# shenwei356/wfa

Measured on AMD Instinct MI355X. Metric: aligned pairs/sec (and Gcells/s) on 1e6 synthetic 1 kbp pairs @5% error, higher is better.
Workload: dtype u32; 1 GPU; 1000000 x 1000 bp pairs/GPU @5% error, global gap-affine 4/6/2, wf-adaptive 10/50/1, seed 3; config=c3, pairs_per_gpu=1000000, length=1000, parallelism=pair-sharded x1, ranks_seen_by_collective=1, backend=none (1 GPU), collective_forced=False, status_ok=1000000, setup_steps=0, gather=none (1 GPU), gather_bytes_per_rank_step=0, packed_pairs=1000000, retried_pairs=831

## Files before the change

### wfa_amd/csrc/wfa_duo.hpp

```cpp
#pragma once
#include "wfa_blk.hpp"
#include "wfa_duo_cfg.hpp"
#include "wfa_pk16.hpp"

namespace wfa {

struct DuoRed {
#define WFA_DUO_3(opa, opb, opc)                                                                                    \
    unsigned long long sv;                                                                                          \
    asm volatile("s_nop 1\n\t" opa " %0, %0, %0 " WFA_DPP_CTL_XOR1 "\n\t" opb " %1, %1, %1 " WFA_DPP_CTL_XOR1 "\n\t" opc \
        " %2, %2, %2 " WFA_DPP_CTL_XOR1 "\n\t" opa " %0, %0, %0 " WFA_DPP_CTL_XOR2 "\n\t" opb " %1, %1, %1 "        \
        WFA_DPP_CTL_XOR2 "\n\t" opc " %2, %2, %2 " WFA_DPP_CTL_XOR2 "\n\t" opa " %0, %0, %0 " WFA_DPP_CTL_HMIR "\n\t" \
        opb " %1, %1, %1 " WFA_DPP_CTL_HMIR "\n\t" opc " %2, %2, %2 " WFA_DPP_CTL_HMIR "\n\t"                         \
        "s_and_saveexec_b64 %3, %4\n\t" opa " %0, %0, %0 " WFA_DPP_CTL_MIR "\n\t" opb " %1, %1, %1 " WFA_DPP_CTL_MIR    \
        "\n\t" opc " %2, %2, %2 " WFA_DPP_CTL_MIR "\n\ts_mov_b64 exec, %3"                                            \
        : "+v"(a), "+v"(b), "+v"(c), "=&s"(sv)                                                                      \
        : "s"(wm)                                                                                                   \
        : "scc");
#define WFA_DUO_2(opa, opb)                                                                                         \
    unsigned long long sv;                                                                                          \
    asm volatile("s_nop 1\n\t" opa " %0, %0, %0 " WFA_DPP_CTL_XOR1 "\n\t" opb " %1, %1, %1 " WFA_DPP_CTL_XOR1 "\n\ts_nop 0\n\t" \
        opa " %0, %0, %0 " WFA_DPP_CTL_XOR2 "\n\t" opb " %1, %1, %1 " WFA_DPP_CTL_XOR2 "\n\ts_nop 0\n\t" opa        \
        " %0, %0, %0 " WFA_DPP_CTL_HMIR "\n\t" opb " %1, %1, %1 " WFA_DPP_CTL_HMIR "\n\t"                            \
        "s_and_saveexec_b64 %2, %3\n\t" opa " %0, %0, %0 " WFA_DPP_CTL_MIR "\n\t" opb " %1, %1, %1 " WFA_DPP_CTL_MIR    \
// ... 29 lines not shown
__device__ __attribute__((always_inline)) inline void duo_run(const KParams &P) {
    constexpr int PP = 4;
    static_assert(DX >= 1 && DOE >= 1 && DX <= 4 && DOE <= 4, "ring depths of one to four score steps");
    constexpr int R  = DX > DOE ? DX : DOE;
    constexpr int RW = PK ? 2 : PP;
    extern __shared__ __attribute__((aligned(16))) uint32_t lds[];
    const int  lane = threadIdx.x, l7 = lane & 7, l15 = lane & 15;
    const bool hi_half = (lane & 8) != 0;

    const uint32_t  SW = P.lds_seq_words, PW = P.prepack_words;
    const uint32_t  FP = duo_fetch_pairs(PW), NBUF = duo_bufs(PW);
    uint32_t *const park0 = lds + NBUF * PW;
    const uint64_t  cap      = P.arena_words;
    const int       mdd      = (int)P.max_dist_diff;
    const int       minwf    = (int)P.min_wf_len;
    const bool      adaptive = P.adaptive != 0;
    const uint32_t  seed_si  = P.dx;
    uint32_t        pk_one   = 0x00010001u;
    if constexpr (PK) asm volatile("" : "+s"(pk_one));
    const int       rows_cap = (int)(cap / 32);

    int       st = 0;
    bool      wide = false;
    uint32_t  pidx = 0, si = 0, cells = 0, sbuf = 0;
    int       n = 0, m = 0, kb = 0;
    bool      slow = false, first_eq = false;
    int             j = l7, k0 = 0;
    uint32_t        mdn = 0u, mup = 0u;
    const uint32_t *lq = lds + 4, *lt = lds + 4;
    uint32_t       *rowp = nullptr;

    uint32_t M[R][RW], I[RW], D[RW];
    int      rlo[R], rhi[R];
    int      lim[PP], lmx[PP];
#pragma unroll
    for (int d = 0; d < R; d++) {
        rlo[d] = BK_BIG, rhi[d] = -BK_BIG;
#pragma unroll
        for (int p = 0; p < RW; p++) M[d][p] = 0u;
    }
#pragma unroll
    for (int p = 0; p < RW; p++) I[p] = D[p] = 0u;
#pragma unroll
    for (int p = 0; p < PP; p++) lim[p] = 0, lmx[p] = 0;

    uint32_t buf_free  = (1u << NBUF) - 1u;
    uint32_t park_used = 0u;
    constexpr uint32_t PF_TOK = 1u, PF_LD = 2u, PF_STAGED = 4u, PF_DRY = 8u;
    uint32_t pf = 0u;
    uint32_t pf_tok = 0u, pf_ld_idx = 0u, pf_idx = 0u, pf_buf = 0u;
    uint32_t st_mask = 0u;
    uint4    pf_w = make_uint4(0u, 0u, 0u, 0u);

#ifdef WFA_STAMPS
    unsigned long long stamp_acc[8] = {0, 0, 0, 0, 0, 0, 0, 0}, stamp_prev;
    unsigned long long evt[16] = {0, 0, 0, 0, 0, 0, 0, 0, 0, 0, 0, 0, 0, 0, 0, 0};
    asm volatile("s_memtime %0\n\ts_waitcnt lgkmcnt(0)" : "=s"(stamp_prev)::"memory");
#endif
    const auto pair_of = [&](uint32_t idx) { return P.work ? P.work[idx] : P.chunk_first + idx; };
    const auto dn1 = [&](uint32_t x) { return (uint32_t)__builtin_amdgcn_update_dpp(0, (int)x, 0x111, 0xf, 0xf, true) & mdn; };
    const auto up1 = [&](uint32_t x) { return (uint32_t)__builtin_amdgcn_update_dpp(0, (int)x, 0x101, 0xf, 0xf, true) & mup; };
    const auto other_half = [&](int x) { return __builtin_amdgcn_update_dpp(0, x, 0x128, 0xf, 0xf, true); };
    const auto set_derived = [&]() {
        j   = wide ? l15 : l7;
        mdn = j == 0 ? 0u : ~0u;
        mup = j == (wide ? 15 : 7) ? 0u : ~0u;
        k0  = kb + PP * j;
#pragma unroll
        for (int p = 0; p < PP; p++) lim[p] = imax2(1, imin2(n + k0 + p, m)), lmx[p] = imax2(n + k0 + p, m);
        lq   = lds + sbuf * PW + 4u;
        lt   = lq + SW;
        if constexpr (DUO_ARENA_FMT == 10u)
            rowp = P.arena + (uint64_t)pidx * cap + (((uint32_t)k0 & 56u) >> 3) * (uint32_t)(rows_cap * 4) + (((uint32_t)k0 >> 2) & 1u) * 16u;
        else if constexpr (DUO_ARENA_FMT == 9u)
            rowp = P.arena + (uint64_t)pidx * cap + (((uint32_t)k0 & 60u) >> 2) * (uint32_t)(rows_cap * 2) + si * 2u;
        else
            rowp = P.arena + (uint64_t)pidx * cap + (uint64_t)(si >> 3) * 256u + (si & 7u) * 2u;
    };
    const auto clear_rings = [&]() {
#pragma unroll
        for (int d = 0; d < R; d++) {
            rlo[d] = BK_BIG, rhi[d] = -BK_BIG;
#pragma unroll
            for (int p = 0; p < RW; p++) M[d][p] = 0u;
        }
#pragma unroll
        for (int p = 0; p < RW; p++) I[p] = D[p] = 0u;
    };
    const auto or_halves = [&](uint32_t v) {
        uint32_t r = 0u;
#pragma unroll
        for (int o = 0; o < 8; o++) r |= (uint32_t)__builtin_amdgcn_readlane((int)v, 8 * o);
        return r;
    };

    const auto refill = [&](auto ph_c) __attribute__((always_inline)) -> bool {
        constexpr int ph  = decltype(ph_c)::value;
        constexpr int NEW = (ph + R - 1) % R;
        pf        = (uint32_t)__builtin_amdgcn_readfirstlane((int)pf);
        park_used = (uint32_t)__builtin_amdgcn_readfirstlane((int)park_used);
        buf_free  = (uint32_t)__builtin_amdgcn_readfirstlane((int)buf_free);
        st_mask   = (uint32_t)__builtin_amdgcn_readfirstlane((int)st_mask);
        if ((pf & (PF_LD | PF_STAGED)) == PF_LD) {
            const uint32_t cnt = umin2(FP, P.chunk_n - pf_ld_idx);
            st_mask = 0u;
            {
                uint32_t f = buf_free;
                for (uint32_t c = 0; c < cnt; c++) st_mask |= f & (0u - f), f &= f - 1u;
            }
            buf_free &= ~st_mask;
            const uint32_t w0 = (uint32_t)lane * 4u, slot = w0 / PW;
            if (slot < cnt) {
                uint32_t f = st_mask;
                for (uint32_t c = 0; c < slot; c++) f &= f - 1u;
                const uint32_t b = (uint32_t)__builtin_ctz(f);
                *reinterpret_cast<uint4 *>(lds + b * PW + (w0 - slot * PW)) = pf_w;
            }
            pf_idx = pf_ld_idx, pf = (pf | PF_STAGED) & ~PF_LD;
        }
        if ((pf & (PF_TOK | PF_LD)) == PF_TOK) {
            pf_ld_idx = (uint32_t)__builtin_amdgcn_readfirstlane((int)pf_tok);
            const bool have = pf_ld_idx < P.chunk_n;
            if (have) {
                const uint32_t *const slot = P.prepack + (uint64_t)pf_ld_idx * PW;
                const uint32_t cnt = umin2(FP, P.chunk_n - pf_ld_idx);
                if ((uint32_t)lane * 4u < cnt * PW) pf_w = *reinterpret_cast<const uint4 *>(slot + lane * 4);
            }
            pf = (pf & ~PF_TOK) | (have ? PF_LD : PF_DRY);
        }
        if ((pf & (PF_TOK | PF_DRY)) == 0u) {
            if (lane == 0) pf_tok = atomicAdd(P.queue_head, FP);
            pf |= PF_TOK;
        }
        unsigned long long m_free;
        WFA_STAMP(0);
        for (;;) {
        const bool run   = st == 1;
        const int  Wc    = wide ? 64 : 32;
        const bool touch = run && rhi[NEW] >= rlo[NEW] && (rlo[NEW] <= kb || rhi[NEW] >= kb + Wc - 1);
        bool       narrowable = false;
        if constexpr (ph == 0) {
            int ulo = rlo[0], uhi = rhi[0];
#pragma unroll
            for (int d = 1; d < R; d++) ulo = imin2(ulo, rlo[d]), uhi = imax2(uhi, rhi[d]);
            narrowable    = run && wide && uhi - ulo + 1 <= DUO_NARROW_AT;
        }
        const unsigned long long m_ev = __ballot(touch || narrowable);
        m_free = __ballot(st == 0);
        if (__builtin_expect(!(m_ev != 0ull || (m_free != 0ull && (park_used != 0u || (pf & PF_STAGED) != 0u))), 1)) break;
        WFA_EVT(1, 1);
        {
            int ulo = rlo[0], uhi = rhi[0];
#pragma unroll
            for (int d = 1; d < R; d++) ulo = imin2(ulo, rlo[d]), uhi = imax2(uhi, rhi[d]);
            const int span = uhi - ulo + 1;
            int act = 0;
            if (touch) act = wide ? (span > DUO_WIDE_MAX ? 4 : 1) : (span > DUO_WIDEN_AT ? 2 : 1);
            else if (narrowable) act = 3;
            const int Wn  = act == 2 ? 64 : (act == 3 ? 32 : Wc);
            const int kbn = (((ulo + uhi + 1 - Wn) >> 1) + 2) & ~3;
            if (act != 0 && act != 4 && !(ulo - kbn >= 1 && uhi - kbn <= Wn - 2)) act = 4;
            const int  o_act = other_half(act), o_kb = other_half(kb), o_kbn = other_half(kbn);
            const bool o_wide = other_half(wide ? 1 : 0) != 0;
            bool widen  = act == 2 && !(hi_half && o_act == 2);
            bool taken  = !wide && !o_wide && o_act == 2 && !(!hi_half && act == 2);
            bool evict  = taken && st == 1;
            unsigned long long m_evict = __ballot(evict);
            bool               lost    = false;
            while (m_evict != 0ull) {
                const int      l0   = __builtin_ctzll(m_evict);
                const uint32_t oct  = (uint32_t)l0 >> 3;
                m_evict &= ~(0xFFull << (8 * oct));
                const bool mine = evict && ((uint32_t)lane >> 3) == oct;
                if (park_used == (1u << DUO_PARK) - 1u) {
                    if (((uint32_t)lane >> 3) == (oct ^ 1u)) lost = true;
                    if (mine) evict = false, taken = false;
                    continue;
                }
                const uint32_t rec = (uint32_t)__builtin_ctz(~park_used);
                park_used |= 1u << rec;
                WFA_EVT(3, 1);
                uint32_t *const pr = park0 + rec * DUO_PARK_WORDS;
                if (mine) {
                    uint4 *const w = reinterpret_cast<uint4 *>(pr + 12 * l7);
                    const auto pk  = [](uint32_t lo, uint32_t hi) { return lo | (hi << 16); };
                    const auto pk2 = [&](const uint32_t(&v)[RW], int h) -> uint32_t {
                        if constexpr (PK) return v[h];
                        else return pk(v[2 * h], v[2 * h + 1]);
                    };
                    uint32_t pw[8];
                    int      plo[4], phi[4];
#pragma unroll
                    for (int r = 0; r < 4; r++) {
                        pw[2 * r]     = r < R ? pk2(M[(ph + r) % R], 0) : 0u;
                        pw[2 * r + 1] = r < R ? pk2(M[(ph + r) % R], 1) : 0u;
                        plo[r] = r < R ? rlo[(ph + r) % R] : BK_BIG, phi[r] = r < R ? rhi[(ph + r) % R] : -BK_BIG;
                    }
                    w[0] = make_uint4(pw[0], pw[1], pw[2], pw[3]);
                    if constexpr (R > 2) w[1] = make_uint4(pw[4], pw[5], pw[6], pw[7]);
                    w[2] = make_uint4(pk2(I, 0), pk2(I, 1), pk2(D, 0), pk2(D, 1));
                    if (l7 == 0) {
                        uint4 *const s4 = reinterpret_cast<uint4 *>(pr + 96);
                        s4[0] = make_uint4(pidx, si, cells, sbuf);
                        s4[1] = make_uint4((uint32_t)n, (uint32_t)m, (uint32_t)kb, (slow ? 1u : 0u) | (first_eq ? 2u : 0u));
                        s4[2] = make_uint4((uint32_t)plo[0], (uint32_t)plo[1], (uint32_t)plo[2], (uint32_t)plo[3]);
                        s4[3] = make_uint4((uint32_t)phi[0], (uint32_t)phi[1], (uint32_t)phi[2], (uint32_t)phi[3]);
                    }
                }
            }
            if (lost) widen = false, act = 4;
            {
                const bool o_lost = other_half(lost ? 1 : 0) != 0;
                if (o_lost) taken = false;
            }
            if (__ballot(act == 4) != 0ull) {
                WFA_EVT(7, __builtin_popcountll(__ballot(act == 4 && j == 0)));
                if (act == 4 && j == 0) {
                    P.pair_meta[pidx] = make_uint4(ST_REDO_BAND, 0u, 0u, 0u);
                    push_redo(P, pair_of(pidx), ST_REDO_BAND);
                }
                buf_free |= or_halves(act == 4 ? (1u << sbuf) : 0u);
                if (act == 4) {
                    st = 0, wide = false;
                    clear_rings();
                }
            }
            const int  rb   = lane & ~15;
            const bool join = taken;
            int src = lane;
            bool moved = false, freed = false;
            {
                if (join) {
                    const int Bo = (lane & ~7) ^ 8, dl = (o_kbn - o_kb) >> 2, jo = (lane - rb) + dl;
                    src = (jo >= 0 && jo < 8) ? Bo + jo : -1, moved = true;
                } else if (act == 1) {
                    const int Bo = wide ? rb : (lane & ~7), Go = wide ? 16 : 8, dl = (kbn - kb) >> 2, jo = (lane - Bo) + dl;
                    src = (jo >= 0 && jo < Go) ? Bo + jo : -1, moved = true;
                } else if (widen) {
                    const int Bo = lane & ~7, dl = (kbn - kb) >> 2, jo = (lane - rb) + dl;
                    src = (jo >= 0 && jo < 8) ? Bo + jo : -1, moved = true;
                } else if (act == 3) {
                    const int dl = (kbn - kb) >> 2, jo = (lane - rb) + dl;
                    if (hi_half) src = -1, freed = true;
                    else src = (jo >= 0 && jo < 16) ? rb + jo : -1;
                    moved = true;
                }
            }
            if (__ballot(moved) != 0ull) {
                WFA_EVT(2, 1);
                const int sl = (src < 0 ? lane : src) << 2;
#pragma unroll
                for (int d = 0; d < R; d++)
#pragma unroll
                    for (int p = 0; p < RW; p++) {
                        const uint32_t v = (uint32_t)__builtin_amdgcn_ds_bpermute(sl, (int)M[d][p]);
                        M[d][p]          = src < 0 ? 0u : v;
                    }
#pragma unroll
                for (int p = 0; p < RW; p++) {
                    const uint32_t v = (uint32_t)__builtin_amdgcn_ds_bpermute(sl, (int)I[p]);
                    const uint32_t u = (uint32_t)__builtin_amdgcn_ds_bpermute(sl, (int)D[p]);
                    I[p] = src < 0 ? 0u : v, D[p] = src < 0 ? 0u : u;
                }
                if (__ballot(join) != 0ull) {
                    const int      o_n = other_half(n), o_m = other_half(m);
                    const uint32_t o_pidx = (uint32_t)other_half((int)pidx), o_si = (uint32_t)other_half((int)si);
                    const uint32_t o_cells = (uint32_t)other_half((int)cells), o_sbuf = (uint32_t)other_half((int)sbuf);
                    const int      o_fl = other_half((slow ? 1 : 0) | (first_eq ? 2 : 0));
                    int o_rlo[R], o_rhi[R];
#pragma unroll
                    for (int d = 0; d < R; d++) o_rlo[d] = other_half(rlo[d]), o_rhi[d] = other_half(rhi[d]);
                    if (join) {
                        n = o_n, m = o_m, pidx = o_pidx, si = o_si, cells = o_cells, sbuf = o_sbuf;
                        slow = (o_fl & 1) != 0, first_eq = (o_fl & 2) != 0;
#pragma unroll
                        for (int d = 0; d < R; d++) rlo[d] = o_rlo[d], rhi[d] = o_rhi[d];
                        st = 1;
                    }
                }
                if (join) kb = o_kbn;
                else if (moved && !freed) kb = kbn;
                if (join || widen) wide = true;
                if (act == 3) wide = false;
                if (freed) {
                    st = 0;
#pragma unroll
                    for (int d = 0; d < R; d++) rlo[d] = BK_BIG, rhi[d] = -BK_BIG;
                }
            }
            m_free = __ballot(st == 0);
            while (m_free != 0ull && (park_used != 0u || (pf & PF_STAGED) != 0u)) {
                const uint32_t oct  = (uint32_t)__builtin_ctzll(m_free) >> 3;
                const bool     mine = ((uint32_t)lane >> 3) == oct;
                if (park_used != 0u) {
                    const uint32_t rec = (uint32_t)__builtin_ctz(park_used);
                    park_used &= park_used - 1u;
                    WFA_EVT(4, 1);
                    const uint32_t *const pr = park0 + rec * DUO_PARK_WORDS;
                    if (mine) {
                        const uint4 *const w = reinterpret_cast<const uint4 *>(pr + 12 * l7);
                        const uint4 v0 = w[0], v1 = R > 2 ? w[1] : make_uint4(0u, 0u, 0u, 0u), v2 = w[2];
                        const uint32_t pw[8] = {v0.x, v0.y, v0.z, v0.w, v1.x, v1.y, v1.z, v1.w};
                        const uint4 *const s4 = reinterpret_cast<const uint4 *>(pr + 96);
                        const uint4 a0 = s4[0], a1 = s4[1], a2 = s4[2], a3 = s4[3];
                        const uint32_t plo[4] = {a2.x, a2.y, a2.z, a2.w}, phi[4] = {a3.x, a3.y, a3.z, a3.w};
#pragma unroll
                        for (int r = 0; r < R; r++) {
                            if constexpr (PK) {
                                M[(ph + r) % R][0] = pw[2 * r], M[(ph + r) % R][1] = pw[2 * r + 1];
                            } else {
                                M[(ph + r) % R][0] = pw[2 * r] & 0xFFFFu, M[(ph + r) % R][1] = pw[2 * r] >> 16;
                                M[(ph + r) % R][2] = pw[2 * r + 1] & 0xFFFFu, M[(ph + r) % R][3] = pw[2 * r + 1] >> 16;
                            }
                            rlo[(ph + r) % R] = (int)plo[r], rhi[(ph + r) % R] = (int)phi[r];
                        }
                        if constexpr (PK) {
                            I[0] = v2.x, I[1] = v2.y, D[0] = v2.z, D[1] = v2.w;
                        } else {
                            I[0] = v2.x & 0xFFFFu, I[1] = v2.x >> 16, I[2] = v2.y & 0xFFFFu, I[3] = v2.y >> 16;
                            D[0] = v2.z & 0xFFFFu, D[1] = v2.z >> 16, D[2] = v2.w & 0xFFFFu, D[3] = v2.w >> 16;
                        }
                        pidx = a0.x, si = a0.y, cells = a0.z, sbuf = a0.w;
                        n = (int)a1.x, m = (int)a1.y, kb = (int)a1.z, slow = (a1.w & 1u) != 0u, first_eq = (a1.w & 2u) != 0u;
                        st = 1, wide = false;
                    }
                    m_free &= ~(0xFFull << (8 * oct));
                    continue;
                }
                pf_buf   = (uint32_t)__builtin_ctz(st_mask);
                st_mask &= st_mask - 1u;
                const uint32_t this_idx = pf_idx;
                pf_idx += 1u;
                const uint32_t *const hb = lds + pf_buf * PW;
                const uint32_t nq = (uint32_t)__builtin_amdgcn_readfirstlane((int)hb[0]), mt = (uint32_t)__builtin_amdgcn_readfirstlane((int)hb[1]);
                const uint32_t status = (uint32_t)__builtin_amdgcn_readfirstlane((int)hb[2]);
                if (st_mask == 0u) pf &= ~PF_STAGED;
                if (status != ST_PENDING) {
                    if (lane == 0) {
                        P.pair_meta[this_idx] = make_uint4(status, 0u, 0u, 0u);
                        if (status >= ST_REDO_BYTES) push_redo(P, pair_of(this_idx), status);
                    }
                    buf_free |= 1u << pf_buf;
                    continue;
                }
                WFA_EVT(5, 1);
                if (mine) {
                    pidx = this_idx, sbuf = pf_buf;
                    n = (int)nq, m = (int)mt;
                    const int Ak = m - n;
                    si = 0, cells = 0, slow = false;
                    kb = -16 + PP * imax2(-3, imin2(3, Ak / (2 * PP)));
                    first_eq = ((hb[4] ^ hb[4 + SW]) & 3u) == 0u;
                    clear_rings();
                    st = 1, wide = false;
                }
                m_free &= ~(0xFFull << (8 * oct));
            }
            set_derived();
            __builtin_amdgcn_fence(__ATOMIC_RELEASE, "wavefront");
            __builtin_amdgcn_fence(__ATOMIC_ACQUIRE, "wavefront");
        }
        }
        WFA_STAMP(1);
        return m_free == ~0ull && park_used == 0u && (pf & (PF_DRY | PF_LD | PF_STAGED)) == PF_DRY;
    };

    const auto step = [&](auto ph_c) __attribute__((always_inline)) {
        constexpr int ph = decltype(ph_c)::value;
        const bool run = (st == 1);
        const unsigned long long wm = __ballot(wide);
        WFA_EVT(0, 1), WFA_EVT(6, __builtin_popcountll(__ballot(run)) / 8);

        uint32_t(&Mo)[RW] = M[(ph + R - DOE) % R];
        uint32_t(&Mx)[RW] = M[(ph + R - DX) % R];
        uint32_t(&Mn)[RW] = M[ph];

        uint32_t nM[PP], nI[RW], nD[RW], wd[RW], cc[PP];
        const uint32_t a_edge = dn1(Mo[RW - 1]), b_edge = dn1(I[RW - 1]);
        const uint32_t c_edge = up1(Mo[0]), d_edge = up1(D[0]);
        const bool     slow_any = __ballot(run && slow) != 0ull;
        const auto next_slow = [&](const uint32_t(&Mo4)[PP], const uint32_t(&I4)[PP], const uint32_t(&D4)[PP], const uint32_t(&Mx4)[PP],
                                   uint32_t ae, uint32_t be, uint32_t ce, uint32_t de, uint32_t(&nI4)[PP], uint32_t(&nD4)[PP],
                                   uint32_t(&wd4)[PP]) __attribute__((always_inline)) {
#pragma unroll
            for (int p = 0; p < PP; p++) {
                const int      k  = k0 + p;
                const uint32_t a0 = p ? Mo4[p - 1] : ae, b0 = p ? I4[p - 1] : be;
                const uint32_t c0 = p < PP - 1 ? Mo4[p + 1] : ce, d0 = p < PP - 1 ? D4[p + 1] : de;
                const uint32_t x0 = Mx4[p];
                const uint32_t a = (int)a0 > m ? 0u : a0, b = (int)b0 > m ? 0u : b0;
                const uint32_t c = (int)c0 - k > n ? 0u : c0, d = (int)d0 - k > n ? 0u : d0;
                const uint32_t x = ((int)x0 > m || (int)x0 - k > n) ? 0u : x0;
                const uint32_t mi = umax2(a, b), tI = umin2(mi, 1u), Isk = mi + tI;
                const uint32_t Dsk = umax2(c, d), tD = umin2(Dsk, 1u);
                const uint32_t x1  = x + umin2(x, 1u);
                const uint32_t Msk = umax3(Isk, Dsk, x1);
                const bool fromX = x != 0u && Msk == x1;
                const bool fromI = !fromX && Msk == Isk;
                const uint32_t mu = umax2(a0, b0), Iu = mu + umin2(mu, 1u), Du = umax2(c0, d0);
                const uint32_t Xu = x0 + umin2(x0, 1u);
                const bool     iext = a < b, dext = c < d;
                const uint32_t o0   = (fromI && iext) ? Iu : ((!fromX && !fromI && dext) ? Du : umax3(Iu, Du, Xu));
                const bool     kin  = k >= -(n - 1) && k <= m - 1;
                nM[p] = kin ? Msk : 0u, nI4[p] = kin ? Isk : 0u, nD4[p] = kin ? Dsk : 0u;
                wd4[p] = blk_word(o0, iext, dext, fromX, fromI);
                cc[p]  = (CENSUS && kin) ? tI + tD + umin2(Msk, 1u) : 0u;
            }
        };
        if constexpr (PK) {
            if (__builtin_expect(!slow_any, 1)) {
                const uint32_t a0 = __builtin_amdgcn_alignbit(Mo[0], a_edge, 16), a1 = __builtin_amdgcn_alignbit(Mo[1], Mo[0], 16);
                const uint32_t c1 = __builtin_amdgcn_alignbit(c_edge, Mo[1], 16);
                const uint32_t b0 = __builtin_amdgcn_alignbit(I[0], b_edge, 16), b1 = __builtin_amdgcn_alignbit(I[1], I[0], 16);
                const uint32_t d0 = __builtin_amdgcn_alignbit(D[1], D[0], 16), d1 = __builtin_amdgcn_alignbit(d_edge, D[1], 16);
                uint32_t M2[2];
                wide_next2<true>(wide_pk(a0), wide_pk(b0), wide_pk(a1) , wide_pk(d0), wide_pk(Mx[0]), wide_pk(pk_one),
                                  M2[0], nI[0], nD[0], wd[0]);
                wide_next2<true>(wide_pk(a1), wide_pk(b1), wide_pk(c1), wide_pk(d1), wide_pk(Mx[1]), wide_pk(pk_one), M2[1], nI[1], nD[1], wd[1]);
#pragma unroll
                for (int p = 0; p < PP; p++) {
                    const int sh = 16 * (p & 1);
                    nM[p] = (M2[p >> 1] >> sh) & 0xFFFFu;
                    cc[p] = CENSUS ? (((nI[p >> 1] >> sh) & 0xFFFFu) != 0u ? 1u : 0u) + (((nD[p >> 1] >> sh) & 0xFFFFu) != 0u ? 1u : 0u) +
                                         (nM[p] != 0u ? 1u : 0u)
// ... 94 lines not shown
            }
#pragma unroll
            for (int p = 0; p < PP; p++) nz[p] = nM[p] != 0u;
        } else {
            unsigned long long cm[PP];
#pragma unroll
            for (int p = 0; p < PP; p++) {
                int h = (int)nM[p];
                nz[p] = h != 0;
                asm("" : "+v"(h));
                uint32_t rem;
                asm("v_sub_u32_e64 %0, %1, %2 clamp" : "=v"(rem) : "v"(lim[p]), "v"(h));
                const uint32_t room = nz[p] ? rem : 0u;
                const int      v    = h - (k0 + p);
                const uint32_t xr   = SeqView<0>::win16(lq, v) ^ SeqView<0>::win16(lt, h);
                const uint32_t rn   = umin2(ffbl_raw(xr) >> 1, room);
                nM[p] = (uint32_t)h + umin2(rn, 16u);
                cm[p] = __builtin_amdgcn_ballot_w64(rn > 16u);
            }
            static_assert(PP == 4, "candidate masks of four diagonals");
            unsigned long long pend = cm[0] | cm[1] | cm[2] | cm[3];
            if (pend != 0ull) WFA_EVT(8, 1);
            while (pend != 0ull) {
                WFA_EVT(9, 1);
                const unsigned long long s0 = cm[0], s1 = cm[1] & ~cm[0], s2 = cm[2] & ~(cm[0] | cm[1]), s3 = cm[3] & ~(cm[0] | cm[1] | cm[2]);
                const bool sel[PP] = {__builtin_amdgcn_inverse_ballot_w64(s0), __builtin_amdgcn_inverse_ballot_w64(s1),
                                      __builtin_amdgcn_inverse_ballot_w64(s2), __builtin_amdgcn_inverse_ballot_w64(s3)};
                uint32_t h  = sel[PP - 1] ? nM[PP - 1] : 0u;
                int      kd = k0 + PP - 1;
#pragma unroll
                for (int p = PP - 2; p >= 0; p--) h = sel[p] ? nM[p] : h, kd = sel[p] ? k0 + p : kd;
                const uint32_t lm = __builtin_amdgcn_inverse_ballot_w64(pend) ? (uint32_t)imin2(n + kd, m) : 0u;
                unsigned long long go;
                do {
                    WFA_EVT(10, 1);
                    const uint2    wq = SeqView<0>::win32(lq, (int)h - kd), wt = SeqView<0>::win32(lt, (int)h);
                    const uint32_t b  = umin2(ffbl_raw(wq.x ^ wt.x), ffbl_raw(wq.y ^ wt.y) | 32u);
                    const uint32_t t  = umin2(umin2(b >> 1, lm - h), 32u);
                    h += t;
                    go = __builtin_amdgcn_ballot_w64(t == 32u);
                } while (go != 0ull);
#pragma unroll
                for (int p = 0; p < PP; p++) nM[p] = sel[p] ? h : nM[p];
                cm[0] &= ~s0, cm[1] &= ~s1, cm[2] &= ~s2, cm[3] &= ~s3;
                pend = cm[0] | cm[1] | cm[2] | cm[3];
            }
        }
        WFA_STAMP(3);

        bool hit[PP], hitl = false;
#pragma unroll
        for (int p = 0; p < PP; p++) hit[p] = nM[p] >= (uint32_t)lim[p], hitl |= hit[p];
        bool       term    = false;
        const bool hit_any = __ballot(hitl) != 0ull;
        bool       ghit    = false;
        if (hit_any) {
            bool tl = false;
#pragma unroll
            for (int p = 0; p < PP; p++) tl |= (k0 + p == m - n && nz[p] && (int)nM[p] >= m);
            const int r = DuoRed::or1((hitl ? 1 : 0) | (tl ? 2 : 0), wm);
            ghit = (r & 1) != 0;
            slow |= ghit;
            term = run && (r & 2) != 0;
        }

        int      ilo = 0, ihi = -1;
        bool     anyM = false;
        uint32_t csum = 0u;
        if (__builtin_expect(!hit_any, 1)) {
            constexpr int ABSENT = BK_BIG + 1;
            int glo = BK_BIG, ghi = -BK_BIG, dd[PP];
#pragma unroll
            for (int p = PP - 1; p >= 0; p--) glo = nz[p] ? PP * j + p : glo;
#pragma unroll
            for (int p = 0; p < PP; p++) {
                ghi   = nz[p] ? PP * j + p : ghi;
                dd[p] = nz[p] ? lmx[p] - (int)nM[p] : ABSENT;
            }
            static_assert(PP == 4, "minimum of four distances");
            int mind = imin2(imin2(dd[0], dd[1]), imin2(dd[2], dd[3]));
            DuoRed::min_max_min(glo, ghi, mind, wm);
            anyM = ghi >= 0;
            const bool want = run && adaptive && anyM && (ghi - glo + 1) >= minwf;
            const int  thr  = want ? mind + mdd : BK_BIG;
            int        first_ok = BK_BIG, last_ok = -BK_BIG;
#pragma unroll
            for (int p = PP - 1; p >= 0; p--) first_ok = dd[p] <= thr ? PP * j + p : first_ok;
#pragma unroll
            for (int p = 0; p < PP; p++) last_ok = dd[p] <= thr ? PP * j + p : last_ok;
            DuoRed::min_max(first_ok, last_ok, wm);
            ilo = first_ok, ihi = last_ok;
#pragma unroll
            for (int p = 0; p < PP; p++) {
                const int  ix   = PP * j + p;
                const bool keep = ix >= ilo && ix <= ihi;
                nM[p] = keep ? nM[p] : 0u;
                if constexpr (!PK) nI[p] = keep ? nI[p] : 0u, nD[p] = keep ? nD[p] : 0u;
                csum += keep ? cc[p] : 0u;
            }
        } else {
            int glo = BK_BIG, ghi = -BK_BIG;
#pragma unroll
            for (int p = PP - 1; p >= 0; p--) glo = nz[p] ? PP * j + p : glo;
#pragma unroll
            for (int p = 0; p < PP; p++) ghi = nz[p] ? PP * j + p : ghi;
            DuoRed::min_max(glo, ghi, wm);
            anyM = ghi >= 0;
// ... 16 lines not shown
                const int  thr   = mind + mdd;
                const bool found = want_reduce && mind != BK_BIG && maxd > thr;
                if (__ballot(found) != 0ull) {
                    int first_ok = BK_BIG, last_ok = -BK_BIG;
#pragma unroll
                    for (int p = PP - 1; p >= 0; p--) first_ok = (vd[p] && dd[p] <= thr) ? PP * j + p : first_ok;
#pragma unroll
                    for (int p = 0; p < PP; p++) last_ok = (vd[p] && dd[p] <= thr) ? PP * j + p : last_ok;
                    DuoRed::min_max(first_ok, last_ok, wm);
                    int leadp = -1;
#pragma unroll
                    for (int p = 0; p < PP; p++) leadp = (vd[p] && PP * j + p < first_ok) ? PP * j + p : leadp;
                    leadp = DuoRed::max1(leadp, wm);
                    const int newlo = ghit ? (leadp >= 0 ? leadp + 1 : glo) : first_ok;
                    if (found) ilo = newlo, ihi = last_ok;
                    csum = 0u;
#pragma unroll
                    for (int p = 0; p < PP; p++) {
                        const int  ix   = PP * j + p;
                        const bool keep = ix >= ilo && ix <= ihi;
                        nM[p] = keep ? nM[p] : 0u;
                        if constexpr (!PK) nI[p] = keep ? nI[p] : 0u, nD[p] = keep ? nD[p] : 0u;
                        csum += keep ? cc[p] : 0u;
                    }
                }
            }
        }

        WFA_STAMP(4);
        const bool keepl = anyM && ihi >= ilo && !no_room;
        if constexpr (CENSUS) {
            int cs = (int)csum, dummy = 0;
            DuoRed::max_add(dummy, cs, wm);
            cells += keepl ? (uint32_t)cs : 0u;
        }
        if constexpr (DUO_ARENA_FMT != 10u) rowp += 2;
        if constexpr (DUO_ARENA_FMT == 7u) rowp += (((uint32_t)(uintptr_t)rowp & 0x38u) == 0u) ? 240 : 0;

        if constexpr (PK) {
#pragma unroll
            for (int h = 0; h < 2; h++) {
                Mn[h] = nM[2 * h] | (nM[2 * h + 1] << 16);
                I[h]  = wide_u32(__builtin_elementwise_min(wide_pk(nI[h]), wide_pk(Mn[h])));
                D[h]  = wide_u32(__builtin_elementwise_min(wide_pk(nD[h]), wide_pk(Mn[h])));
            }
        } else {
#pragma unroll
            for (int p = 0; p < PP; p++) Mn[p] = nM[p], I[p] = nI[p], D[p] = nD[p];
        }
        rlo[ph] = keepl ? kb + ilo : BK_BIG;
        rhi[ph] = keepl ? kb + ihi : -BK_BIG;

        const bool fin = run && (term || no_room);
        if (__ballot(fin) != 0ull) {
            const int ctot = (CENSUS && P.census) ? (int)cells : 0;
            int hf   = 0;
#pragma unroll
            for (int p = 0; p < PP; p++)
                if (k0 + p == m - n) hf = (int)nM[p];
            hf = DuoRed::max1(hf, wm);
            if (fin && j == 0) {
                if (no_room) {
                    P.pair_meta[pidx] = make_uint4(ST_REDO_ARENA, 0u, 0u, 0u);
                    push_redo(P, pair_of(pidx), ST_REDO_ARENA);
                } else {
                    P.pair_meta[pidx] = make_uint4(ST_OK, si * P.g, (uint32_t)hf, (uint32_t)ctot);
                }
            }
            buf_free |= or_halves(fin ? (1u << sbuf) : 0u);
            if (fin) {
                st = 0, wide = false;
                clear_rings();
            }
        }
        if (run && !fin) si += 1u;
        WFA_STAMP(5);
    };

    for (;;) {
        if (refill(std::integral_constant<int, 0>{})) break;
        step(std::integral_constant<int, 0>{});
        if constexpr (R > 1) {
            if (refill(std::integral_constant<int, 1 % R>{})) break;
            step(std::integral_constant<int, 1 % R>{});
        }
        if constexpr (R > 2) {
            if (refill(std::integral_constant<int, 2 % R>{})) break;
            step(std::integral_constant<int, 2 % R>{});
        }
        if constexpr (R > 3) {
            if (refill(std::integral_constant<int, 3 % R>{})) break;
            step(std::integral_constant<int, 3 % R>{});
        }
    }
#ifdef WFA_STAMPS
    if (lane == 0 && P.debug_info) {
        unsigned long long *acc = reinterpret_cast<unsigned long long *>(P.debug_info);
        for (int i = 0; i < 8; i++) atomicAdd(acc + i, stamp_acc[i]);
        for (int i = 0; i < 16; i++) atomicAdd(acc + 8 + i, evt[i]);
    }
#endif
}

#ifndef WFA_DUO_VGPRS
#define WFA_DUO_VGPRS 64
#endif
static_assert(16u * (256u - 4u) / 2u < 2048u, "wfa_duo_kernel's packed rings need offsets under 4 096");
template <bool CENSUS, int DX = 2, int DOE = 4>
__global__ __launch_bounds__(64, WFA_DUO_WAVES) __attribute__((amdgpu_num_vgpr(WFA_DUO_VGPRS))) void wfa_duo_kernel(const KParams P) {
    duo_run<CENSUS, DX, DOE, true>(P);
}
template <bool CENSUS, int DX = 2, int DOE = 4>
__global__ __launch_bounds__(64, WFA_DUO_WAVES) __attribute__((amdgpu_num_vgpr(WFA_DUO_VGPRS))) void wfa_duo32_kernel(const KParams P) {
    duo_run<CENSUS, DX, DOE, false>(P);
}

}
```

### wfa_amd/csrc/wfa_duo_cfg.hpp

```cpp
#pragma once
#include "wfa_common.hpp"

namespace wfa {

#ifndef WFA_DUO_WAVES
#define WFA_DUO_WAVES 4
#endif
#ifndef WFA_DUO_PARK
#define WFA_DUO_PARK 4
#endif
#ifndef WFA_DUO_WIDEN_AT
#define WFA_DUO_WIDEN_AT 26
#endif
#ifndef WFA_DUO_NARROW_AT
#define WFA_DUO_NARROW_AT 21
#endif
#ifndef WFA_DUO_GROUP_MAJOR
#define WFA_DUO_GROUP_MAJOR 2
#endif
#ifndef WFA_DUO_EXTEND
#define WFA_DUO_EXTEND 1
#endif
constexpr uint32_t DUO_ARENA_FMT = WFA_DUO_GROUP_MAJOR == 2 ? 10u : WFA_DUO_GROUP_MAJOR == 1 ? 9u : 7u;
constexpr int DUO_PARK       = WFA_DUO_PARK;
constexpr int DUO_PARK_WORDS = 8 * 12 + 16;
constexpr int DUO_BUFS       = 8 + 1 + DUO_PARK;
constexpr int DUO_FETCH_MAX  = 8;
constexpr int DUO_WIDEN_AT   = WFA_DUO_WIDEN_AT;
constexpr int DUO_NARROW_AT  = WFA_DUO_NARROW_AT;
constexpr int DUO_WIDE_MAX   = 56;

__host__ __device__ inline uint32_t duo_fetch_pairs(uint32_t prepack_words) {
    const uint32_t f = 256u / prepack_words;
    return f < 1u ? 1u : (f > (uint32_t)DUO_FETCH_MAX ? (uint32_t)DUO_FETCH_MAX : f);
}
__host__ __device__ inline uint32_t duo_bufs(uint32_t prepack_words) { return 8u + duo_fetch_pairs(prepack_words) + (uint32_t)DUO_PARK; }
__host__ __device__ inline uint32_t duo_lds_words(uint32_t prepack_words) {
    return duo_bufs(prepack_words) * prepack_words + (uint32_t)DUO_PARK * DUO_PARK_WORDS;
}

hipError_t wfa_launch_duo(int shape, const KParams &P, uint32_t grid, size_t lds_bytes, hipStream_t st, bool census, bool pk);

}
```

### wfa_amd/csrc/wfa_host.hip

```cpp
#include <map>
#include "wfa_ctx.hpp"
#include "wfa_bound.hpp"
#include "wfa_generic.hpp"
#include "wfa_packed.hpp"
#include "wfa_reg.hpp"
#include "wfa_blk.hpp"
#include "wfa_duo_cfg.hpp"
#include "wfa_lane.hpp"
#include "wfa_team.hpp"
#include "wfa_teamc.hpp"
#include "wfa_fwd.hpp"
#include "wfa_long.hpp"
#include "wfa_wide.hpp"

using namespace wfa;
static_assert(TEAM_SOLO_MAX == 4096, "wfa_ctx.hpp: default of opt_team_solo_max");

namespace wfa {
hipError_t wfa_launch_fwd(int shape, int kind, uint32_t flags, const KParams &P, uint32_t grid, size_t lds_bytes, hipStream_t st) {
    switch (shape) {
    case 0: return wfa_launch_fwd_s24(kind, flags, P, grid, lds_bytes, st);
    case 1: return wfa_launch_fwd_s13(kind, flags, P, grid, lds_bytes, st);
    case 2: return wfa_launch_fwd_s12(kind, flags, P, grid, lds_bytes, st);
    case 3: return wfa_launch_fwd_s23(kind, flags, P, grid, lds_bytes, st);
// ... 1093 lines not shown
                    if (rc) return rc;
                    ctx->timing.n_packed_pairs += (uint32_t)(lst.size() - r2.size());
                    keep.insert(keep.end(), r2.begin(), r2.end());
                    redo1.swap(keep);
                    if (wide_ok) {
                        const int wv = wide_pass(redo1);
                        if (wv < 0) return wv;
                    }
                }
            }
            redo1.insert(redo1.end(), redo_w.begin(), redo_w.end());
            redo_w.clear();
            if (kind1 >= 2 && can_b && !wide_ok && redo1.size() > resident_generic) {
                std::vector<uint32_t> lst;
                for (uint64_t e : redo1) {
                    const uint32_t stw = (uint32_t)(e >> 32);
                    if (stw == ST_REDO_BYTES) jb.pairs.push_back((uint32_t)e);
                    else if (stw == ST_REDO_BAND) lst.push_back((uint32_t)e);
                    else ja.pairs.push_back((uint32_t)e);
                }
                if (!lst.empty()) {
                    if ((rc = forward_pass(1, &lst, 0, lst.size(), redo2, false))) return rc;
                    ctx->timing.n_packed_pairs += (uint32_t)(lst.size() - redo2.size());
                    for (uint64_t e : redo2) ((uint32_t)(e >> 32) == ST_REDO_BYTES ? jb : ja).pairs.push_back((uint32_t)e);
                }
            } else {
                for (uint64_t e : redo1) ((uint32_t)(e >> 32) == ST_REDO_BYTES ? jb : ja).pairs.push_back((uint32_t)e);
            }
            if (skip_rest)
                for (uint64_t i = done_pairs; i < n_pairs; i++) ja.pairs.push_back((uint32_t)i);
            std::sort(ja.pairs.begin(), ja.pairs.end());
            for (Job *jp : {&ja, &jb}) {
                if (jp->pairs.empty()) continue;
                if (sub_len_used == 0) {
                    jobs.push_back(std::move(*jp));
                    continue;
                }
                Job js = *jp, jl = *jp;
                js.pairs.clear(), jl.pairs.clear();
                js.max_len = sub_len_used;
                for (uint32_t pid : jp->pairs) (h_len[pid] <= sub_len_used ? js : jl).pairs.push_back(pid);
                if (!js.pairs.empty()) jobs.push_back(std::move(js));
                if (!jl.pairs.empty()) jobs.push_back(std::move(jl));
            }
#ifdef WFA_STAMPS
            {
                unsigned long long acc[24];
                HIP_TRY(hipMemcpy(acc, P.debug_info, 192, hipMemcpyDeviceToHost));
                std::fprintf(stderr, "[events] wave-steps %llu  slow %llu  hit %llu  reduce %llu  found %llu  found pair-steps %llu  "
                             "continuation iterations %llu  running pair-steps %llu\n", acc[8], acc[9], acc[10], acc[11], acc[12],
                             acc[13], acc[14], acc[15]);
                std::fprintf(stderr, "[duo extend] wave-steps into the continuation %llu  outer rounds %llu  inner rounds %llu\n", acc[16], acc[17],
                             acc[18]);
                unsigned long long tot = 0;
                for (int i = 0; i < 6; i++) tot += acc[i];
                const char *nm[6] = {"refill", "next", "extend", "ranges+reduce", "stores", "ring+finish+window"};
                for (int i = 0; i < 6; i++)
                    std::fprintf(stderr, "[stamps] %-22s %6.2f %%  (%llu cyc)\n", nm[i], 100.0 * acc[i] / (double)tot, acc[i]);
                P.debug_info = nullptr;
            }
#endif
            if (ctx->band_key == rkey && ctx->band_kind == 9 && mid_in > 0 && mid_fail * 2 > mid_in) ctx->band_kind = 5;
            first       = false;
            packed_done = true;
        }
    }
    uint64_t  lkey = 0;
    {
        uint32_t lb = 0;
        while ((2u << lb) <= max_len) lb++;
        lkey = 1ull | ((uint64_t)lb << 1) | ((uint64_t)(ctx->opt_team_compact != 0) << 7) | ((uint64_t)P.global_alignment << 8) | ((uint64_t)P.adaptive << 9) | ((uint64_t)(P.x & 0xFFF) << 12) |
               ((uint64_t)(P.oe & 0xFFF) << 24) | ((uint64_t)(P.e & 0xFFF) << 36) | ((uint64_t)(P.max_dist_diff & 0xFFFF) << 48);
    }
    int      learned_now = -1;
    uint64_t team_total = 0, team_done = 0;
    const bool learn_track = !packed_done && ctx->opt_team_min_len > 0 && max_len >= (uint64_t)ctx->opt_team_min_len;
    if (!packed_done) {
        Job j;
        j.mode = ctx->force_mode == 1 ? 1 : 0, j.level = 0, j.all = true;
        if (ctx->opt_learn && !debug_single && ctx->learn_key == lkey && ctx->opt_team_min_len > 0 && max_len >= (uint64_t)ctx->opt_team_min_len) {
            j.level = ctx->learn_level;
            if (j.level > 0 && (++ctx->learn_calls & 15u) == 0u) j.level -= 1;
            j.hint = j.level > 0;
        }
        j.scout = true;
        ctx->timing.ladder_start_level = (uint32_t)j.level;
        jobs.push_back(std::move(j));
    }

    while (!jobs.empty()) {
        ctrl_fresh = false, ctrl_zeroed = false;
        Job job = std::move(jobs.front());
        jobs.pop_front();
        const uint64_t n_work = job.all ? n_pairs : job.pairs.size();
        if (n_work == 0) continue;
        const uint32_t max_len_all = max_len;
        const uint32_t max_len     = job.max_len ? job.max_len : max_len_all;
        LaunchCfg cfg;
        int       cr = make_cfg(ctx, max_len, job.mode, job.level, n_work, !P.global_alignment, cfg);
        if (cr == 1) {
            job.mode = 1;
            cr       = make_cfg(ctx, max_len, 1, job.level, n_work, !P.global_alignment, cfg);
        }
        while (cr == 2 && job.hint && job.level > 0) {
            job.level -= 1;
            cr = make_cfg(ctx, max_len, job.mode, job.level, n_work, !P.global_alignment, cfg);
// ... 391 lines not shown
```

Baseline: 67.26 million pairs/s.

## Precompute wave event masks at step end to skip the between-steps window loop

New measurement: 67.13 million pairs/s. Within noise of the previous version (-0.2%).

```diff
diff --git a/wfa_amd/csrc/wfa_duo.hpp b/wfa_amd/csrc/wfa_duo.hpp
--- a/wfa_amd/csrc/wfa_duo.hpp
+++ b/wfa_amd/csrc/wfa_duo.hpp
@@ -105,9 +105,23 @@
     uint32_t st_mask = 0u;
     uint4    pf_w = make_uint4(0u, 0u, 0u, 0u);
 
+    unsigned long long h_touch = 0ull, h_free = ~0ull, h_wide = 0ull;
+
 #ifdef WFA_STAMPS
-    unsigned long long stamp_acc[8] = {0, 0, 0, 0, 0, 0, 0, 0}, stamp_prev;
-    unsigned long long evt[16] = {0, 0, 0, 0, 0, 0, 0, 0, 0, 0, 0, 0, 0, 0, 0, 0};
+    uint32_t           stamp_lane = 0u, evt_lane = 0u;
+    unsigned long long stamp_prev;
+#undef WFA_STAMP
+#undef WFA_EVT
+#define WFA_STAMP(i)                                                                \
+    do {                                                                            \
+        unsigned long long _t;                                                      \
+        __builtin_amdgcn_sched_barrier(0);                                          \
+        asm volatile("s_memtime %0\n\ts_waitcnt lgkmcnt(0)" : "=s"(_t)::"memory"); \
+        __builtin_amdgcn_sched_barrier(0);                                          \
+        stamp_lane += lane == (i) ? (uint32_t)(_t - stamp_prev) : 0u;               \
+        stamp_prev = _t;                                                            \
+    } while (0)
+#define WFA_EVT(i, v) (evt_lane += lane == (i) ? (uint32_t)(v) : 0u)
     asm volatile("s_memtime %0\n\ts_waitcnt lgkmcnt(0)" : "=s"(stamp_prev)::"memory");
 #endif
     const auto pair_of = [&](uint32_t idx) { return P.work ? P.work[idx] : P.chunk_first + idx; };
@@ -187,36 +201,62 @@
         }
         unsigned long long m_free;
         WFA_STAMP(0);
+        if constexpr (WFA_DUO_BETWEEN != 0) {
+            unsigned long long m_ev0 = h_touch;
+            if constexpr (ph == 0) {
+                if (h_wide != 0ull) {
+                    int ulo = rlo[0], uhi = rhi[0];
+#pragma unroll
+                    for (int d = 1; d < R; d++) ulo = imin2(ulo, rlo[d]), uhi = imax2(uhi, rhi[d]);
+                    m_ev0 |= __builtin_amdgcn_ballot_w64(uhi - ulo + 1 <= DUO_NARROW_AT) & h_wide & ~h_free;
+                }
+            }
+            if (__builtin_expect(!(m_ev0 != 0ull || (h_free != 0ull && (park_used != 0u || (pf & PF_STAGED) != 0u))), 1)) {
+                WFA_STAMP(1);
+                return h_free == ~0ull && park_used == 0u && (pf & (PF_DRY | PF_LD | PF_STAGED)) == PF_DRY;
+            }
+        }
+#ifdef WFA_STAMPS
+        bool again = false;
+#endif
         for (;;) {
         const bool run   = st == 1;
         const int  Wc    = wide ? 64 : 32;
+        int        ulo = rlo[0], uhi = rhi[0];
+#pragma unroll
+        for (int d = 1; d < R; d++) ulo = imin2(ulo, rlo[d]), uhi = imax2(uhi, rhi[d]);
+        const int  span  = uhi - ulo + 1;
         const bool touch = run && rhi[NEW] >= rlo[NEW] && (rlo[NEW] <= kb || rhi[NEW] >= kb + Wc - 1);
-        bool       narrowable = false;
-        if constexpr (ph == 0) {
-            int ulo = rlo[0], uhi = rhi[0];
-#pragma unroll
-            for (int d = 1; d < R; d++) ulo = imin2(ulo, rlo[d]), uhi = imax2(uhi, rhi[d]);
-            narrowable    = run && wide && uhi - ulo + 1 <= DUO_NARROW_AT;
-        }
+        const bool narrowable = ph == 0 && run && wide && span <= DUO_NARROW_AT;
         const unsigned long long m_ev = __ballot(touch || narrowable);
         m_free = __ballot(st == 0);
         if (__builtin_expect(!(m_ev != 0ull || (m_free != 0ull && (park_used != 0u || (pf & PF_STAGED) != 0u))), 1)) break;
         WFA_EVT(1, 1);
+#ifdef WFA_STAMPS
+        WFA_EVT(14, again ? 1 : 0);
+        again = true;
+#endif
+        WFA_EVT(11, m_ev == 0ull ? 1 : 0);
         {
-            int ulo = rlo[0], uhi = rhi[0];
-#pragma unroll
-            for (int d = 1; d < R; d++) ulo = imin2(ulo, rlo[d]), uhi = imax2(uhi, rhi[d]);
-            const int span = uhi - ulo + 1;
             int act = 0;
+            int kbn = kb;
+            if (WFA_DUO_BETWEEN == 0 || m_ev != 0ull) {
             if (touch) act = wide ? (span > DUO_WIDE_MAX ? 4 : 1) : (span > DUO_WIDEN_AT ? 2 : 1);
             else if (narrowable) act = 3;
             const int Wn  = act == 2 ? 64 : (act == 3 ? 32 : Wc);
-            const int kbn = (((ulo + uhi + 1 - Wn) >> 1) + 2) & ~3;
+            kbn = (((ulo + uhi + 1 - Wn) >> 1) + 2) & ~3;
             if (act != 0 && act != 4 && !(ulo - kbn >= 1 && uhi - kbn <= Wn - 2)) act = 4;
-            const int  o_act = other_half(act), o_kb = other_half(kb), o_kbn = other_half(kbn);
+            }
+            WFA_EVT(12, m_ev != 0ull && __builtin_amdgcn_ballot_w64(act > 1) == 0ull ? 1 : 0), WFA_EVT(13, __builtin_amdgcn_ballot_w64(act > 1) != 0ull ? 1 : 0);
+            const bool any_widen = WFA_DUO_BETWEEN == 0 || __builtin_amdgcn_ballot_w64(act == 2) != 0ull;
+            int        o_kb = 0, o_kbn = 0;
+            bool       widen = false, taken = false;
+            if (any_widen) {
+            const int  o_act = other_half(act);
             const bool o_wide = other_half(wide ? 1 : 0) != 0;
-            bool widen  = act == 2 && !(hi_half && o_act == 2);
-            bool taken  = !wide && !o_wide && o_act == 2 && !(!hi_half && act == 2);
+            o_kb = other_half(kb), o_kbn = other_half(kbn);
+            widen       = act == 2 && !(hi_half && o_act == 2);
+            taken       = !wide && !o_wide && o_act == 2 && !(!hi_half && act == 2);
             bool evict  = taken && st == 1;
             unsigned long long m_evict = __ballot(evict);
             bool               lost    = false;
@@ -266,6 +306,7 @@
                 const bool o_lost = other_half(lost ? 1 : 0) != 0;
                 if (o_lost) taken = false;
             }
+            }
             if (__ballot(act == 4) != 0ull) {
                 WFA_EVT(7, __builtin_popcountll(__ballot(act == 4 && j == 0)));
                 if (act == 4 && j == 0) {
@@ -282,14 +323,15 @@
             const bool join = taken;
             int src = lane;
             bool moved = false, freed = false;
-            {
-                if (join) {
+            const auto ring_src = [&](auto jw_c) __attribute__((always_inline)) {
+                constexpr bool jw = decltype(jw_c)::value;
+                if (jw && join) {
                     const int Bo = (lane & ~7) ^ 8, dl = (o_kbn - o_kb) >> 2, jo = (lane - rb) + dl;
                     src = (jo >= 0 && jo < 8) ? Bo + jo : -1, moved = true;
                 } else if (act == 1) {
                     const int Bo = wide ? rb : (lane & ~7), Go = wide ? 16 : 8, dl = (kbn - kb) >> 2, jo = (lane - Bo) + dl;
                     src = (jo >= 0 && jo < Go) ? Bo + jo : -1, moved = true;
-                } else if (widen) {
+                } else if (jw && widen) {
                     const int Bo = lane & ~7, dl = (kbn - kb) >> 2, jo = (lane - rb) + dl;
                     src = (jo >= 0 && jo < 8) ? Bo + jo : -1, moved = true;
                 } else if (act == 3) {
@@ -298,7 +340,9 @@
                     else src = (jo >= 0 && jo < 16) ? rb + jo : -1;
                     moved = true;
                 }
-            }
+            };
+            if (any_widen) ring_src(std::true_type{});
+            else if (m_ev != 0ull) ring_src(std::false_type{});
             if (__ballot(moved) != 0ull) {
                 WFA_EVT(2, 1);
                 const int sl = (src < 0 ? lane : src) << 2;
@@ -315,7 +359,7 @@
                     const uint32_t u = (uint32_t)__builtin_amdgcn_ds_bpermute(sl, (int)D[p]);
                     I[p] = src < 0 ? 0u : v, D[p] = src < 0 ? 0u : u;
                 }
-                if (__ballot(join) != 0ull) {
+                if (any_widen && __ballot(join) != 0ull) {
                     const int      o_n = other_half(n), o_m = other_half(m);
                     const uint32_t o_pidx = (uint32_t)other_half((int)pidx), o_si = (uint32_t)other_half((int)si);
                     const uint32_t o_cells = (uint32_t)other_half((int)cells), o_sbuf = (uint32_t)other_half((int)sbuf);
@@ -342,6 +386,8 @@
                 }
             }
             m_free = __ballot(st == 0);
+        }
+        {
             while (m_free != 0ull && (park_used != 0u || (pf & PF_STAGED) != 0u)) {
                 const uint32_t oct  = (uint32_t)__builtin_ctzll(m_free) >> 3;
                 const bool     mine = ((uint32_t)lane >> 3) == oct;
@@ -422,7 +468,7 @@
         constexpr int ph = decltype(ph_c)::value;
         const bool run = (st == 1);
         const unsigned long long wm = __ballot(wide);
-        WFA_EVT(0, 1), WFA_EVT(6, __builtin_popcountll(__ballot(run)) / 8);
+        WFA_EVT(0, 1), WFA_EVT(6, __builtin_popcountll(__ballot(run)) / 8), WFA_EVT(15, wm == 0ull ? 1 : 0);
 
         uint32_t(&Mo)[RW] = M[(ph + R - DOE) % R];
         uint32_t(&Mx)[RW] = M[(ph + R - DX) % R];
@@ -623,7 +669,10 @@
 #pragma unroll
         for (int p = 0; p < PP; p++) hit[p] = nM[p] >= (uint32_t)lim[p], hitl |= hit[p];
         bool       term    = false;
-        const bool hit_any = __ballot(hitl) != 0ull;
+        static_assert(PP == 4, "end tests of four diagonals");
+        const bool hit_any = WFA_DUO_BETWEEN != 0 ? (__builtin_amdgcn_ballot_w64(hit[0]) | __builtin_amdgcn_ballot_w64(hit[1]) |
+                                                     __builtin_amdgcn_ballot_w64(hit[2]) | __builtin_amdgcn_ballot_w64(hit[3])) != 0ull
+                                                  : __ballot(hitl) != 0ull;
         bool       ghit    = false;
         if (hit_any) {
             bool tl = false;
@@ -746,6 +795,14 @@
         rhi[ph] = keepl ? kb + ihi : -BK_BIG;
 
         const bool fin = run && (term || no_room);
+        if constexpr (WFA_DUO_BETWEEN != 0) {
+            const unsigned long long m_run = __builtin_amdgcn_ballot_w64(run), m_fin = __builtin_amdgcn_ballot_w64(fin);
+            const unsigned long long m_edge = __builtin_amdgcn_ballot_w64(ilo <= 0) | __builtin_amdgcn_ballot_w64(ihi >= 63) |
+                                              (__builtin_amdgcn_ballot_w64(ihi >= 31) & ~wm);
+            h_touch = m_edge & __builtin_amdgcn_ballot_w64(keepl) & m_run & ~m_fin;
+            h_free  = ~m_run | m_fin;
+            h_wide  = wm & ~m_fin;
+        }
         if (__ballot(fin) != 0ull) {
             const int ctot = (CENSUS && P.census) ? (int)cells : 0;
             int hf   = 0;
@@ -788,10 +845,10 @@
         }
     }
 #ifdef WFA_STAMPS
-    if (lane == 0 && P.debug_info) {
+    if (lane < 16 && P.debug_info) {
         unsigned long long *acc = reinterpret_cast<unsigned long long *>(P.debug_info);
-        for (int i = 0; i < 8; i++) atomicAdd(acc + i, stamp_acc[i]);
-        for (int i = 0; i < 16; i++) atomicAdd(acc + 8 + i, evt[i]);
+        if (lane < 8) atomicAdd(acc + lane, (unsigned long long)stamp_lane);
+        atomicAdd(acc + 8 + lane, (unsigned long long)evt_lane);
     }
 #endif
 }
diff --git a/wfa_amd/csrc/wfa_duo_cfg.hpp b/wfa_amd/csrc/wfa_duo_cfg.hpp
--- a/wfa_amd/csrc/wfa_duo_cfg.hpp
+++ b/wfa_amd/csrc/wfa_duo_cfg.hpp
@@ -21,6 +21,9 @@
 #ifndef WFA_DUO_EXTEND
 #define WFA_DUO_EXTEND 1
 #endif
+#ifndef WFA_DUO_BETWEEN
+#define WFA_DUO_BETWEEN 1
+#endif
 constexpr uint32_t DUO_ARENA_FMT = WFA_DUO_GROUP_MAJOR == 2 ? 10u : WFA_DUO_GROUP_MAJOR == 1 ? 9u : 7u;
 constexpr int DUO_PARK       = WFA_DUO_PARK;
 constexpr int DUO_PARK_WORDS = 8 * 12 + 16;
diff --git a/wfa_amd/csrc/wfa_host.hip b/wfa_amd/csrc/wfa_host.hip
--- a/wfa_amd/csrc/wfa_host.hip
+++ b/wfa_amd/csrc/wfa_host.hip
@@ -1169,6 +1169,8 @@
                              acc[13], acc[14], acc[15]);
                 std::fprintf(stderr, "[duo extend] wave-steps into the continuation %llu  outer rounds %llu  inner rounds %llu\n", acc[16], acc[17],
                              acc[18]);
+                std::fprintf(stderr, "[duo rounds] no event, free halves only %llu  recentre only %llu  with widen / narrow / hand-on %llu  "
+                             "second and later iterations %llu  wave-steps without a wide pair %llu\n", acc[19], acc[20], acc[21], acc[22], acc[23]);
                 unsigned long long tot = 0;
                 for (int i = 0; i < 6; i++) tot += acc[i];
                 const char *nm[6] = {"refill", "next", "extend", "ranges+reduce", "stores", "ring+finish+window"};
```
